# aarchiiive/diff-unet-amos

Hardware: AMD Instinct MI355X
Metric: denoised voxel-steps/sec on 96^3 16-class AMOS patches (higher is better)
Workload: dtype f16

## Files before the change

diff_unet_amos_amd/_native.py:

```python
from __future__ import annotations

import ctypes as C
import os

import torch

_HERE = os.path.dirname(os.path.abspath(__file__))
LIB_PATH = os.path.join(_HERE, "libdua_hip.so")
if os.environ.get("DUA_DEBUG") == "1" and os.environ.get("DUA_HIP_LIB"):
    LIB_PATH = os.environ["DUA_HIP_LIB"]

F32, F16 = 0, 1
U8 = 2
ERR_ARG = -22
SURFACE_FIELDS = ("hd", "hd95", "asd", "assd", "tp", "fp", "fn", "tn", "hd95_lo", "hd95_hi", "asd_ba", "n_surface")


class NativeLibraryMissing(RuntimeError):
    pass


class Conv3Desc(C.Structure):
    _fields_ = [("dtype", C.c_int), ("N", C.c_int), ("D", C.c_int), ("H", C.c_int), ("W", C.c_int),
                ("Cin", C.c_int), ("Cin_stride", C.c_int), ("Cin_off", C.c_int),
# ... 71 lines not shown
                ("out", C.c_void_p), ("ldc", C.c_int), ("out_off", C.c_int), ("x", C.c_void_p),
                ("stats", C.c_void_p), ("c_pad", C.c_int), ("geom", WindowGeom), ("gamma", C.c_void_p), ("beta", C.c_void_p),
                ("eps", C.c_float), ("ln_out", C.c_void_p), ("background", C.c_int)]


TOKLIN_PLAIN, TOKLIN_GELU, TOKLIN_STATS, TOKLIN_RESIDUAL, TOKLIN_SCATTER = range(5)

TEMB_MAX_BLOCKS, ADAMW_MAX_TENSORS = 16, 64


class TembBlocks(C.Structure):
    _fields_ = [("nblocks", C.c_int), ("cout", C.c_int * TEMB_MAX_BLOCKS), ("w", C.c_void_p * TEMB_MAX_BLOCKS),
                ("b", C.c_void_p * TEMB_MAX_BLOCKS), ("dw", C.c_void_p * TEMB_MAX_BLOCKS), ("db", C.c_void_p * TEMB_MAX_BLOCKS)]


class PackItem(C.Structure):
    _fields_ = [("kind", C.c_int), ("Cout", C.c_int), ("Cin", C.c_int), ("packed", C.c_int), ("w", C.c_void_p), ("out", C.c_void_p)]


class AdamWList(C.Structure):
    _fields_ = [("count", C.c_int), ("numel", C.c_long * ADAMW_MAX_TENSORS), ("p", C.c_void_p * ADAMW_MAX_TENSORS),
                ("g", C.c_void_p * ADAMW_MAX_TENSORS), ("m", C.c_void_p * ADAMW_MAX_TENSORS), ("v", C.c_void_p * ADAMW_MAX_TENSORS)]

class AugVolume(C.Structure):
    _fields_ = [("image", C.c_void_p), ("label", C.c_void_p), ("fg_prefix", C.c_void_p), ("bg_prefix", C.c_void_p),
                ("D", C.c_int), ("H", C.c_int), ("W", C.c_int), ("nchunks", C.c_int), ("fg_count", C.c_uint),
                ("bg_count", C.c_uint), ("image_threshold", C.c_float), ("reserved", C.c_int)]


class AugConfig(C.Structure):
    _fields_ = [("roi", C.c_int * 3), ("max_k", C.c_int), ("pos_fraction", C.c_float), ("flip_prob", C.c_float),
                ("rot90_prob", C.c_float), ("scale_prob", C.c_float), ("scale_factors", C.c_float), ("shift_prob", C.c_float),
                ("shift_offsets", C.c_float), ("reserved", C.c_int)]


class AugSmoothing(C.Structure):
    _fields_ = [("alpha", C.c_float), ("order", C.c_float), ("epsilon", C.c_float), ("max_value", C.c_float)]


AUG_CHUNK, AUG_MAX_CLASSES, AUG_PARAM_WORDS = 1024, 64, 8
AUG_VOLUME, AUG_START_D, AUG_START_H, AUG_START_W, AUG_FLIP, AUG_K, AUG_SCALE, AUG_SHIFT = range(8)

_P = C.c_void_p
ABI_VERSION = 8

_SIGS = {
    "dua_abi_version": (C.c_int, []),
    "dua_prepare": (C.c_int, []),
    "dua_prepared_kernels": (C.c_int, []),
    "dua_mfma_probe": (C.c_int, [C.c_int, C.c_int, _P, _P, _P]),
    "dua_chain_probe": (C.c_int, [C.c_int, C.c_int, _P, _P, _P, _P]),
    "dua_deconv_k2s2_fwd": (C.c_int, [C.POINTER(Conv3Desc), _P, _P, _P, C.POINTER(InNorm), _P, _P]),
    "dua_deconv_k2s2_pad_fwd": (C.c_int, [C.POINTER(Conv3Desc), C.c_int, C.c_int, C.c_int, _P, _P, _P, C.POINTER(InNorm), _P, _P]),
    "dua_conv3d_k3_dgrad_reduce_supported": (C.c_int, [C.POINTER(Conv3Desc)]),
    "dua_conv3d_k3_dgrad_reduce": (C.c_int, [C.POINTER(Conv3Desc), _P, _P, _P, _P, _P, C.c_int, C.c_int, C.POINTER(InNorm), _P, _P]),
    "dua_deconv_k2s2_res_supported": (C.c_int, [C.POINTER(Conv3Desc), C.c_int]),
    "dua_deconv_k2s2_res_fwd": (C.c_int, [C.POINTER(Conv3Desc), _P, _P, _P, C.c_int, C.c_int, C.c_int, _P, _P, _P, _P]),
    "dua_q_sample": (C.c_int, [C.c_int, C.c_long, _P, _P, _P, _P, _P]),
    "dua_sampler_step": (C.c_int, [C.c_int, C.c_int, C.c_long, _P, _P, _P, _P, _P, _P, _P, _P]),
    "dua_final_conv_sampler": (C.c_int, [C.POINTER(TailDesc), _P, C.POINTER(InNorm)] + [_P] * 11),
    "dua_final_conv_sampler_res": (C.c_int, [C.POINTER(TailDesc), _P, C.POINTER(InNorm), C.POINTER(TailResidual)] + [_P] * 11),
    "dua_window_attention_fwd": (C.c_int, [C.c_int, C.c_int, C.c_int, C.c_int, C.c_int, _P, _P, _P, _P, _P, C.c_int, C.c_int, C.c_int,
                                           C.c_float, _P, _P]),
    "dua_patch_merge_norm": (C.c_int, [C.c_int] * 7 + [_P, _P, _P, _P, C.c_float, _P, _P]),
    "dua_residual_norm_act": (C.c_int, [C.c_int, C.c_int, C.c_long, C.c_int, _P, C.c_int, C.POINTER(InNorm), _P, C.c_int,
                                        C.POINTER(InNorm), _P, C.c_int, C.c_int, C.c_float, _P, C.c_int, C.c_int, _P, C.c_int,
                                        C.c_int, C.c_int, _P]),
    "dua_window_gather_norm": (C.c_int, [C.c_int, C.POINTER(WindowGeom), _P, _P, _P, _P, C.c_float, _P, _P]),
    "dua_window_scatter_add_norm": (C.c_int, [C.c_int, C.POINTER(WindowGeom), _P, _P, _P, _P, C.c_float, _P, _P]),
    "dua_stage_out": (C.c_int, [C.c_int, C.c_int, C.c_long, C.c_int, _P, _P, C.c_int, C.c_float, _P, _P, _P, C.c_int, C.c_int, _P]),
    "dua_patch_embed": (C.c_int, [C.c_int] * 8 + [_P, _P, _P, _P, C.c_int, C.c_float, _P, _P, _P, C.c_int, C.c_int, _P]),
    "dua_instnorm_stats": (C.c_int, [C.c_int, C.c_int, C.c_long, C.c_int, _P, C.c_int, C.c_int, _P, C.c_int, _P]),
    "dua_gelu": (C.c_int, [C.c_int, C.c_long, _P, _P]),
    "dua_token_linear": (C.c_int, [C.POINTER(TokenLinearDesc), _P]),
    "dua_token_gemm": (C.c_int, [C.POINTER(TokenLinearDesc), _P, C.c_long, _P]),
    "dua_token_gemm_workspace": (C.c_long, [C.c_long, C.c_int, C.c_int]),
    "dua_swin_mlp": (C.c_int, [C.c_long, C.c_int, _P, _P, _P, _P, _P, _P, _P]),
    "dua_denoiser_step": (C.c_int, [C.POINTER(DenoiserPlan), _P]),
    "dua_temb_table": (C.c_int, [C.c_int, _P, _P, C.c_int, C.c_int, _P, _P, _P, _P, _P, _P, C.c_int, _P, _P]),
    "dua_step_begin": (C.c_int, [C.c_int, C.c_int, _P, C.c_int, _P, _P, C.c_int, _P, _P, _P, _P, _P, _P, _P]),
    "dua_step_begin_clear": (C.c_int, [C.c_int, C.c_int, _P, C.c_int, _P, _P, C.c_int, _P, _P, _P, _P, _P, _P, _P, C.c_long, _P]),
    "dua_conv3d_k3_workspace": (C.c_long, [C.POINTER(Conv3Desc)]),
    "dua_conv3d_k3_kernel_kind": (C.c_int, [C.POINTER(Conv3Desc), C.c_int, C.c_int]),
    "dua_deconv_k2s2_kernel_kind": (C.c_int, [C.POINTER(Conv3Desc)]),
    "dua_conv3d_k3_fwd": (C.c_int, [C.POINTER(Conv3Desc), _P, _P, _P, C.POINTER(InNorm), _P, _P, _P, C.c_long, _P]),
    "dua_upconv_k3_supported": (C.c_int, [C.POINTER(UpConvDesc)]),
    "dua_pack_upconv_weights": (C.c_long, [C.c_int, C.c_int, C.c_int, C.c_int, C.c_int, C.c_int, _P, _P, _P, _P, _P, _P, _P]),
    "dua_upconv_k3_fwd": (C.c_int, [C.POINTER(UpConvDesc), _P, _P, C.POINTER(InNorm), _P, _P, _P, _P, _P, _P]),
    "dua_conv3d_k3_wgrad_workspace": (C.c_long, [C.POINTER(Conv3Desc)]),
    "dua_conv3d_k3_wgrad": (C.c_int, [C.POINTER(Conv3Desc), _P, _P, _P, C.c_int, _P, _P, C.c_long, _P]),
    "dua_pack_conv3_weights": (C.c_long, [C.c_int, C.c_int, C.c_int, C.c_int, _P, _P, _P, _P]),
    "dua_pack_conv3_weights_tap": (C.c_long, [C.c_int, C.c_int, C.c_int, C.c_int, C.c_int, C.c_int, _P, _P, _P, _P]),
    "dua_pack_conv3_weights_dgrad": (C.c_long, [C.c_int, C.c_int, C.c_int, C.c_int, _P, _P, _P]),
    "dua_instnorm_finalize": (C.c_int, [C.c_int, C.c_int, C.POINTER(InNorm), _P, _P, _P]),
    "dua_instnorm_bwd_reduce": (C.c_int, [C.POINTER(NormBwdDesc), _P, _P, C.POINTER(InNorm), _P, _P]),
    "dua_instnorm_bwd_apply": (C.c_int, [C.POINTER(NormBwdDesc), _P, _P, C.POINTER(InNorm), _P, _P, _P, _P, _P, _P]),
    "dua_maxpool2_bwd_add": (C.c_int, [C.c_int] * 6 + [_P, C.c_int, C.c_int, _P, C.c_int, C.c_int, _P, C.c_int, _P, C.c_int, _P]),
    "dua_pack_deconv_weights_dgrad": (C.c_long, [C.c_int, C.c_int, C.c_int, _P, _P, _P]),
    "dua_deconv_k2s2_bwd_workspace": (C.c_long, [C.POINTER(Conv3Desc)]),
    "dua_deconv_k2s2_bwd": (C.c_int, [C.POINTER(Conv3Desc), _P, _P, _P, _P, _P, _P, C.c_long, _P]),
    "dua_deconv_k2s2_pad_bwd": (C.c_int, [C.POINTER(Conv3Desc), C.c_int, C.c_int, C.c_int, _P, _P, _P, _P, _P, _P, C.c_long, _P]),
    "dua_head_fwd": (C.c_int, [C.c_int, C.c_long, C.c_int, C.c_int, _P, C.c_int, _P, _P, _P, C.c_int, _P]),
    "dua_head_bwd_workspace": (C.c_long, [C.c_long]),
    "dua_head_bwd": (C.c_int, [C.c_int, C.c_long, C.c_int, C.c_int, _P, C.c_int, _P, C.c_int, _P, _P, C.c_int, _P, _P, _P, C.c_long, _P]),
    "dua_seg_loss_reduce": (C.c_int, [C.c_int, C.c_int, C.c_int, C.c_long, _P, C.c_int, _P, _P, _P]),
    "dua_seg_loss_grad": (C.c_int, [C.c_int, C.c_int, C.c_int, C.c_long, _P, C.c_int, _P, _P, _P, C.c_float, C.c_float,
                                    C.c_float, _P, C.c_int, _P]),
    "dua_materialize": (C.c_int, [C.POINTER(MaterializeDesc), _P, C.POINTER(InNorm), _P, _P, _P, _P]),
    "dua_pack_deconv_weights": (C.c_long, [C.c_int, C.c_int, C.c_int, _P, _P, _P]),
    "dua_to_channels_last": (C.c_int, [C.c_int, C.c_int, C.c_int, C.c_long, _P, _P, C.c_int, C.c_int, C.c_int, _P]),
    "dua_from_channels_last": (C.c_int, [C.c_int, C.c_int, C.c_int, C.c_long, _P, C.c_int, C.c_int, _P, _P]),
    "dua_pack_conv3_weights_batch": (C.c_int, [C.c_int, C.c_int, C.POINTER(PackItem), _P]),
    "dua_to_channels_last_rows": (C.c_int, [C.c_int, C.c_int, C.c_int, _P, C.c_int, _P, C.c_long, _P, C.c_int, _P]),
    "dua_linear_f32": (C.c_int, [C.c_long, C.c_int, C.c_int, _P, C.c_long, _P, _P, _P, C.c_long, C.c_int, _P]),
    "dua_stats_channel_sums": (C.c_int, [C.c_int, C.c_int, C.c_int, _P, _P, _P]),
    "dua_seg_loss_finish": (C.c_int, [C.c_int, C.c_int, C.c_long, C.c_int, C.c_int, C.c_int, C.c_int, _P, _P, _P, _P]),
    "dua_q_sample_affine": (C.c_int, [C.c_int, C.c_long, _P, C.c_float, C.c_float, _P, _P, C.c_int, _P, _P, _P]),
    "dua_multi_neighbor_columns": (C.c_int, [C.c_int] * 7 + [_P, C.c_int, _P, _P, _P]),
    "dua_multi_neighbor_angles": (C.c_int, [C.c_int, C.c_int, _P, _P, _P]),
    "dua_seg_loss_finish_mn": (C.c_int, [C.c_int, C.c_int, C.c_long, C.c_int, C.c_int, C.c_int, C.c_int, _P, C.c_int, _P, _P, _P,
                                         _P]),
    "dua_temb_train_fwd": (C.c_int, [C.c_int, _P, _P, C.c_int, C.c_int, _P, _P, _P, _P, C.POINTER(TembBlocks), _P, _P, _P]),
    "dua_temb_train_bwd": (C.c_int, [C.c_int, C.c_int, C.c_int, _P, C.POINTER(TembBlocks), _P, _P, _P, _P, _P, _P, _P, _P]),
    "dua_grads_nonfinite": (C.c_int, [C.POINTER(AdamWList), _P, _P]),
    "dua_adamw_step": (C.c_int, [C.POINTER(AdamWList), C.c_float, _P, C.c_float, C.c_float, C.c_float, C.c_float, _P, _P, _P,
                                 C.c_int, _P]),
    "dua_adamw_advance": (C.c_int, [_P, _P, _P, _P, C.c_float, C.c_float, C.c_int, _P, _P]),
    "dua_surface_scratch_bytes": (C.c_long, [C.c_int] * 4),
    "dua_surface_masks": (C.c_int, [C.c_int] * 4 + [_P, C.c_int, C.c_long, _P, C.c_int, C.c_long, C.c_int, _P, C.c_long, _P, _P]),
    "dua_surface_edt_sq": (C.c_int, [C.c_int] * 4 + [_P, C.c_long, C.c_int, C.c_double, C.c_double, C.c_double, _P, _P]),
    "dua_surface_distance_table": (C.c_int, [C.c_int] * 4 + [_P, C.c_int, C.c_long, _P, C.c_int, C.c_long, C.c_int] +
                                   [C.c_double] * 3 + [C.c_int, _P, _P, _P, C.c_long, _P]),
    "dua_aug_count_candidates": (C.c_int, [_P, _P, C.c_long, C.c_float, _P, _P]),
    "dua_aug_draw": (C.c_int, [_P, C.c_int, _P, C.c_int, C.POINTER(AugConfig), C.c_ulonglong, _P, C.c_int, C.c_ulonglong, _P, _P,
                               _P]),
    "dua_aug_apply": (C.c_int, [_P, C.c_int, _P, C.c_int, C.c_int, C.c_int, C.c_int, _P, C.c_int, _P, _P, _P, _P]),
    "dua_aug_class_centroids": (C.c_int, [_P, C.c_int, C.c_int, C.c_int, C.c_int, _P, _P, _P]),
    "dua_aug_apply_smoothed": (C.c_int, [_P, C.c_int, _P, C.c_int, C.POINTER(AugSmoothing), _P, C.c_int, C.c_int, C.c_int, C.c_int,
                                         _P, C.c_int, _P, _P, _P, _P]),
}

_lib = None


def exported_symbols():
    return sorted(_SIGS)


def lib():
    global _lib
    if _lib is None:
        if not os.path.exists(LIB_PATH):
            raise NativeLibraryMissing(
                f"{LIB_PATH} not found: build it with `python -c 'import __graft_entry__ as g; g.build()'` "
                "(hipcc --offload-arch=gfx950). There is no CPU fallback.")
        L = C.CDLL(LIB_PATH)
        for name, (res, args) in _SIGS.items():
            fn = getattr(L, name)
            fn.restype, fn.argtypes = res, args
        got = L.dua_abi_version()
        if got != ABI_VERSION:
            raise NativeLibraryMissing(f"{LIB_PATH} has ABI version {got}, this binding needs {ABI_VERSION}: rebuild the library")
        _lib = L
    return _lib


# ... 29 lines not shown
```

diff_unet_amos_amd/csrc/conv3d_igemm.hip:

```cpp
#include "common.hpp"
#include "../../include/dua_hip.h"
#include "conv3_args.hpp"
#include "stamp.hpp"
#include <algorithm>

namespace dua {

namespace c3 {
constexpr int TD = 4, TH = 8, TW = 8;
constexpr int HD = TD + 2, HH = TH + 2, HW = TW + 2;
constexpr int KG = 4;
constexpr int VS = KG * 16;
constexpr int RS = HW * VS + 16;
constexpr int PS = HH * RS;
constexpr int HALO_BYTES = HD * PS;
constexpr int BN = 64;
}

static inline int conv_variant_of(const dua_conv3_desc* d) { return d->policy & 0xff; }
static inline bool conv_policy_ok(const dua_conv3_desc* d) {
  const int v = d->policy & 0xff;
  return (d->policy & ~(0xff | DUA_POLICY_NO_FINISH)) == 0 && (v == 0 || v == 2 || v == 3 || v == 6 || v == 7 || v == 8 || v == 9);
}

#ifdef DUA_ABLATE
extern int g_wgrad_abl;
#endif

namespace c3v2 {
using namespace c3;
constexpr int SLAB = 3 * KG * BN * 16;
constexpr int LDS_MAIN = HALO_BYTES + 2 * SLAB;
}

__device__ __forceinline__ void glds16(const void* g, void* lds_wave_base) {
  __builtin_amdgcn_global_load_lds((const __attribute__((address_space(1))) void*)g,
                                   (__attribute__((address_space(3))) void*)lds_wave_base, 16, 0, 0);
}

template <typename T, int TDP = 4, int NKS = 2, bool HALF = false, bool BIG = false>
__global__ __launch_bounds__(256, BIG ? 1 : 2) void conv3d_k3_v2_kernel(Conv3Args a) {
  using namespace c3v2;
  constexpr int TD = TDP, HD = TDP + 2, MB = TDP == 2 ? 1 : 2;
  constexpr int NW = 4, NTHR = 64 * NW;
  constexpr int BSLAB = 3 * SLAB;
  constexpr int HALO_BYTES = HD * PS, LDS_MAIN = HALO_BYTES + (BIG ? 3 * BSLAB : 2 * SLAB);
  static_assert(!BIG || (NKS == 2 && !HALF), "the kd-plane form is the plain 32-channel-chunk kernel");
  constexpr int NITEMS = HD * HH * HW * KG, NIT = (NITEMS + NTHR - 1) / NTHR;
  constexpr int NPIECE = SLAB / 16, NSL = (NPIECE + NTHR - 1) / NTHR;
  using Frag = typename Elem<T>::Frag;
  constexpr int EPG = Elem<T>::EPG;
  constexpr int CK = KG * EPG;
  extern __shared__ __attribute__((aligned(16))) char smem[];
  char* halo = smem;
  char* wbuf = smem + HALO_BYTES;
  float* xsc = (float*)(smem + LDS_MAIN);
  float* xsh = xsc + a.nchunks * CK;
  float* xad = xsh + a.nchunks * CK;

  const int tid = threadIdx.x, lane = tid & 63, wave = tid >> 6;
  const int r = lane & 31, hh = lane >> 5;
  const int dwave = TDP == 2 ? wave >> 1 : wave;
  const int hbase = TDP == 2 ? (wave & 1) * 4 : 0;
  const int tile = xcd_remap(blockIdx.x, a.ntiles);
  const int ct = blockIdx.y, n = blockIdx.z % a.N;
  const int tw_ = tile % a.tiles_w, th_ = (tile / a.tiles_w) % a.tiles_h, td_ = tile / (a.tiles_w * a.tiles_h);
  const int d0 = td_ * TD, h0 = th_ * TH, w0 = tw_ * TW;
  const bool fused = a.xf.stats != nullptr;

  const int kg_t = tid & (KG - 1);
  long goff[NIT]; int loff[NIT];
  const T* xin = (const T*)a.x + (long)n * a.D * a.H * a.W * a.Cin_stride + a.Cin_off;
#pragma unroll
  for (int j = 0; j < NIT; ++j) {
    int it = tid + NTHR * j;
    int hv = it >> 2;
    int hd = hv / (HH * HW), rem = hv - hd * (HH * HW), hy = rem / HW, hx = rem - hy * HW;
    int gd = d0 + hd - 1, gh = h0 + hy - 1, gw = w0 + hx - 1;
    bool ok = it < NITEMS && gd >= 0 && gd < a.D && gh >= 0 && gh < a.H && gw >= 0 && gw < a.W;
    goff[j] = ok ? (((long)gd * a.H + gh) * a.W + gw) * a.Cin_stride + kg_t * EPG : -1;
#ifndef DUA_HALO_BRANCHFREE
    loff[j] = it < NITEMS ? hd * PS + hy * RS + hx * VS + kg_t * 16 : -1;
#else
    loff[j] = it < NITEMS ? hd * PS + hy * RS + hx * VS + kg_t * 16 : HW * VS;
#endif
  }
  const char* wsrc = (const char*)a.w + (long)ct * a.nchunks * 9 * SLAB;
  f32x4 wreg[3][NSL];
  auto load_slab = [&](int g, int set) {
    const char* src = wsrc + (long)g * SLAB + tid * 16;
#pragma unroll
    for (int j = 0; j < NSL; ++j)
      if (NPIECE % NTHR == 0 || tid + NTHR * j < NPIECE) wreg[set][j] = *(const f32x4*)(src + j * NTHR * 16);
  };
  auto store_slab = [&](int g, int set) {
    char* dst = wbuf + (g & 1) * SLAB + tid * 16;
#pragma unroll
    for (int j = 0; j < NSL; ++j)
      if (NPIECE % NTHR == 0 || tid + NTHR * j < NPIECE) *(f32x4*)(dst + j * NTHR * 16) = wreg[set][j];
  };
  Frag hv_[NIT];
#ifndef DUA_HALO_BRANCHFREE
  auto load_halo = [&](int ch) {
    const bool cok = ch * CK + kg_t * EPG < a.Cin;
#pragma unroll
// ... 518 lines not shown
        mma32(acc[m][0], ta[m][s], tb[s][0]);
        mma32(acc[m][1], ta[m][s], tb[s][1]);
      }
    if (slot < 56) DUA_STAMP_AT(slot, false);
    __syncthreads();
    if (slot < 56) DUA_STAMP_AT(slot + 1, false);

    char* ot = halo + wave * 4096;
    float* ex = (float*)(smem + LDS_F);
    const int gd = d0 + wave;
    const bool dok = gd < a.D;
    const bool full = d0 + TD <= a.D && h0 + TH <= a.H && w0 + TW <= a.W;
    const long nvox = (long)a.D * a.H * a.W;
    T* yout = (T*)a.y + (long)n * nvox * a.Cout_stride;
    float s[2] = {0.f, 0.f}, ss[2] = {0.f, 0.f};
#pragma unroll
    for (int m = 0; m < MB; ++m) {
      if (full) {
#pragma unroll
        for (int q = 0; q < 2; ++q)
#pragma unroll
          for (int i = 0; i < 16; ++i) {
            const float v = acc[m][q][i];
            s[q] += v;
            ss[q] = fmaf(v, v, ss[q]);
            *(T*)(ot + acc_row(i, hh) * 128 + (q * 32 + r) * 2) = (T)v;
          }
      } else {
#pragma unroll
        for (int q = 0; q < 2; ++q)
#pragma unroll
          for (int i = 0; i < 16; ++i) {
            const int hl = 4 * m + (i >> 2), wl = (i & 3) + 4 * hh;
            const bool ok = dok && (h0 + hl < a.H) && (w0 + wl < a.W);
            const float v = ok ? acc[m][q][i] : 0.f;
            s[q] += v;
            ss[q] = fmaf(v, v, ss[q]);
            *(T*)(ot + acc_row(i, hh) * 128 + (q * 32 + r) * 2) = (T)v;
          }
      }
      __builtin_amdgcn_fence(__ATOMIC_RELEASE, "wavefront");
      __builtin_amdgcn_wave_barrier();
      __builtin_amdgcn_fence(__ATOMIC_ACQUIRE, "wavefront");
      if (dok) {
#pragma unroll
        for (int it = 0; it < 4; ++it) {
          const int v = it * 8 + (lane >> 3), cg = lane & 7;
          const int gh = h0 + 4 * m + (v >> 3), gw = w0 + (v & 7);
          if ((full || (gh < a.H && gw < a.W)) && ct * BN + cg * 8 < a.Cout)
            *(f16x8*)(yout + chan_off(a.out_blk, ((long)gd * a.H + gh) * a.W + gw, a.Cout_off + ct * BN + cg * 8, a.Cout_stride, nvox)) =
                *(const f16x8*)(ot + v * 128 + cg * 16);
        }
      }
      __builtin_amdgcn_fence(__ATOMIC_RELEASE, "wavefront");
      __builtin_amdgcn_wave_barrier();
      __builtin_amdgcn_fence(__ATOMIC_ACQUIRE, "wavefront");
    }
#pragma unroll
    for (int q = 0; q < 2; ++q) {
      s[q] += __shfl_xor(s[q], 32);
      ss[q] += __shfl_xor(ss[q], 32);
      if (hh == 0) { ex[(wave * BN + q * 32 + r) * 2] = s[q]; ex[(wave * BN + q * 32 + r) * 2 + 1] = ss[q]; }
    }
    if (slot < 56) DUA_STAMP_AT(slot + 2, false);
    __syncthreads();
    if (wave == 0) {
      double S = 0, Q = 0;
#pragma unroll
      for (int w = 0; w < NW; ++w) { S += (double)ex[(w * BN + lane) * 2]; Q += (double)ex[(w * BN + lane) * 2 + 1]; }
      if (ct * BN + lane < a.Cout) stats_add(a.stats, n, a.cout_pad, item & (STAT_REPLICAS - 1), ct * BN + lane, S, Q);
    }
    if (more) {
      store_halo();
      __syncthreads();
    }
    if (slot < 56) DUA_STAMP_AT(slot + 3, false);
    slot += 4;
  }
  DUA_STAMP_AT(62, false);
  DUA_STAMP_AT(63, false);
  DUA_STAMP_AT(1, true);
}

template <typename T>
__global__ __launch_bounds__(256) void splitk_finish_kernel(const float* __restrict__ part, int ksplit, int N, long vox,
                                                            int cout_pad, int Cout, const float* __restrict__ bias,
                                                            T* __restrict__ y, int Cout_stride, int Cout_off,
                                                            stat_t* stats, int G, int VL, int ITER) {
  using part_t = typename std::conditional<sizeof(T) == 4, double, float>::type;
  __shared__ part_t red[256][8];
  const int n = blockIdx.y;
  const int cg = threadIdx.x % G, vl = threadIdx.x / G;
  const int c = cg * 4;
  part_t s[4] = {0, 0, 0, 0}, q[4] = {0, 0, 0, 0};
  f32x4 b4 = {0.f, 0.f, 0.f, 0.f};
  if (c < Cout) b4 = *(const f32x4*)(bias + c);
  if (vl < VL && ITER == 2 && ksplit <= 8) {
    const long va = ((long)blockIdx.x * 2) * VL + vl, vb = va + VL;
    const long kstride = (long)N * vox * cout_pad;
    const float* pa = part + ((long)n * vox + (va < vox ? va : 0)) * cout_pad + c;
    const float* pb = part + ((long)n * vox + (vb < vox ? vb : 0)) * cout_pad + c;
    f32x4 qa[8], qb[8];
#pragma unroll
    for (int j = 0; j < 8; ++j) {
      const int kk = j < ksplit ? j : ksplit - 1;
      qa[j] = *(const f32x4*)(pa + kk * kstride);
      qb[j] = *(const f32x4*)(pb + kk * kstride);
    }
    f32x4 acc[2] = {b4, b4};
#pragma unroll
    for (int j = 0; j < 8; ++j)
      if (j < ksplit)
#pragma unroll
        for (int e = 0; e < 4; ++e) { acc[0][e] += qa[j][e]; acc[1][e] += qb[j][e]; }
#pragma unroll
    for (int i = 0; i < 2; ++i) {
      const long v = i ? vb : va;
      if (v >= vox) break;
      T o[4];
#pragma unroll
      for (int e = 0; e < 4; ++e) {
        o[e] = (T)acc[i][e];
        const float f = (float)o[e];
        s[e] += f; q[e] += (part_t)f * (part_t)f;
      }
      if (c < Cout) {
        T* yp = y + ((long)n * vox + v) * Cout_stride + Cout_off + c;
#pragma unroll
        for (int e = 0; e < 4; ++e) yp[e] = o[e];
      }
    }
  } else if (vl < VL) {
    for (int i = 0; i < ITER; ++i) {
      const long v = ((long)blockIdx.x * ITER + i) * VL + vl;
      if (v >= vox) break;
      f32x4 acc = b4;
      const float* pp = part + ((long)n * vox + v) * cout_pad + c;
      const long kstride = (long)N * vox * cout_pad;
      int k = 0;
      for (; k + 16 <= ksplit; k += 16) {
        f32x4 pv[16];
#pragma unroll
        for (int j = 0; j < 16; ++j) pv[j] = *(const f32x4*)(pp + (k + j) * kstride);
#pragma unroll
        for (int j = 0; j < 16; ++j)
#pragma unroll
          for (int e = 0; e < 4; ++e) acc[e] += pv[j][e];
      }
      if (k < ksplit) {
        f32x4 pv[16];
#pragma unroll
        for (int j = 0; j < 16; ++j) {
          const int kk = k + j < ksplit ? k + j : ksplit - 1;
          pv[j] = *(const f32x4*)(pp + kk * kstride);
        }
#pragma unroll
        for (int j = 0; j < 16; ++j)
          if (k + j < ksplit)
#pragma unroll
            for (int e = 0; e < 4; ++e) acc[e] += pv[j][e];
      }
      T o[4];
#pragma unroll
      for (int e = 0; e < 4; ++e) {
        o[e] = (T)acc[e];
        const float f = (float)o[e];
        s[e] += f; q[e] += (part_t)f * (part_t)f;
      }
      if (c < Cout) {
        T* yp = y + ((long)n * vox + v) * Cout_stride + Cout_off + c;
#pragma unroll
        for (int e = 0; e < 4; ++e) yp[e] = o[e];
      }
    }
  }
#pragma unroll
  for (int e = 0; e < 4; ++e) { red[threadIdx.x][e] = s[e]; red[threadIdx.x][4 + e] = q[e]; }
  __syncthreads();
  for (int ch = threadIdx.x; ch < 4 * G; ch += 256) {
    const int g4 = ch >> 2, e = ch & 3;
    double S = 0, Q = 0;
    for (int j = 0; j < VL; ++j) { S += (double)red[j * G + g4][e]; Q += (double)red[j * G + g4][4 + e]; }
    if (ch < Cout) stats_add(stats, n, cout_pad, blockIdx.x & (STAT_REPLICAS - 1), ch, S, Q);
  }
}


static inline void choose_split(int base_wgs, int units, int* ksplit, int* ups, int target = 320, int max_base = 64) {
  *ksplit = 1; *ups = units;
  if (base_wgs > max_base || units <= 1) return;
  int want = target == 320 ? (320 + base_wgs - 1) / base_wgs : target / base_wgs;
  if (want < 1) want = 1;
  if (want > units) want = units;
  *ups = (units + want - 1) / want;
  *ksplit = (units + *ups - 1) / *ups;
}

constexpr int PARTIAL_LDS_PAD = 36 * 1024;

static const LdsAttr kConvLdsAttrs[] = {
    {(const void*)conv3d_k3_v2_kernel<f16, 4>, c3v2::LDS_MAIN + 3 * 4 * 1024 + PARTIAL_LDS_PAD},
    {(const void*)conv3d_k3_v2_kernel<float, 4>, c3v2::LDS_MAIN + 3 * 4 * 1024 + PARTIAL_LDS_PAD},
    {(const void*)conv3d_k3_v2_kernel<f16, 4, 1>, c3v2::LDS_MAIN + 4096 + PARTIAL_LDS_PAD},
    {(const void*)conv3d_k3_v2_kernel<f16, 4, 0>, c3v2::LDS_MAIN + 4096 + PARTIAL_LDS_PAD},
    {(const void*)conv3d_k3_v2_kernel<f16, 4, 2, true>, c3v2::LDS_MAIN + 3 * 4 * 1024 + PARTIAL_LDS_PAD},
    {(const void*)conv3d_k3_first_kernel, c3f::LDS_F + 2048 + PARTIAL_LDS_PAD},
    {(const void*)conv3d_k3_v2_kernel<f16, 2>, c3v2::LDS_MAIN + 3 * 4 * 1024},
    {(const void*)conv3d_k3_v2_kernel<float, 2>, c3v2::LDS_MAIN + 3 * 4 * 1024},
    {(const void*)conv3d_k3_v2_kernel<f16, 4, 2, false, true>, 160 * 1024},
    {(const void*)conv3d_k3_v2_kernel<float, 4, 2, false, true>, 160 * 1024},
    {(const void*)conv3d_k3_v2_kernel<f16, 2, 2, false, true>, 160 * 1024},
    {(const void*)conv3d_k3_v2_kernel<float, 2, 2, false, true>, 160 * 1024},
};
static const LdsAttrs kConvLdsReg(kConvLdsAttrs);

static int conv3_kernel_kind(const dua_conv3_desc* d, bool fused) {
  const int g_conv_variant = conv_variant_of(d);
  if (d->dtype != DUA_F16) return 0;
  if (d->tap_channel_plus1 > 0) return (d->tap_channel_plus1 == 17 && g_conv_variant == 0) ? 1 : 0;
  const long tiles = (long)((d->D + 3) / 4) * ((d->H + 7) / 8) * ((d->W + 7) / 8) * ((d->Cout + c3::BN - 1) / c3::BN) * d->N;
  const long vox = (long)d->D * d->H * d->W;
  if ((g_conv_variant == 0 || g_conv_variant == 8 || g_conv_variant == 9) && !d->background && tiles >= 1024 && d->D % 8 == 0 && d->H % 8 == 0 && d->W % 8 == 0 &&
      d->Cin % 16 == 0 && d->Cin <= (fused ? 256 : 384) && vox * d->Cin_stride < 0x7fffffffL)
    return 2;
  return 0;
}

struct BwdSums { const void* raw; int stride, off; const dua_in_norm* in; double* sums; };

template <typename T>
static int launch_conv3(const dua_conv3_desc* d, const void* x, const void* w, const float* bias,
                        const dua_in_norm* in, void* y, stat_t* stats, float* ws, long ws_bytes, hipStream_t s,
                        const BwdSums* bw = nullptr) {
  using namespace c3;
  constexpr int CK = KG * Elem<T>::EPG;
  Conv3Args a;
  a.x = x; a.w = w; a.bias = bias; a.y = y; a.stats = stats;
  a.bw_raw = nullptr; a.bw_stride = a.bw_off = 0; a.bw_xf = make_xform(nullptr, d->Cout); a.bw_sums = nullptr;
  if (bw) {
    a.bw_raw = bw->raw; a.bw_stride = bw->stride; a.bw_off = bw->off; a.bw_xf = make_xform(bw->in, d->Cout); a.bw_sums = bw->sums;
  }
  a.xf = make_xform(in, d->Cin);
  a.N = d->N; a.D = d->D; a.H = d->H; a.W = d->W;
  a.Cin = d->Cin; a.Cin_stride = d->Cin_stride; a.Cin_off = d->Cin_off;
  a.Cout = d->Cout; a.Cout_stride = d->Cout_stride; a.Cout_off = d->Cout_off;
  a.nchunks = (d->Cin + CK - 1) / CK;
  const int td = (d->D + TD - 1) / TD;
  a.tiles_h = (d->H + TH - 1) / TH; a.tiles_w = (d->W + TW - 1) / TW;
  a.ntiles = td * a.tiles_h * a.tiles_w;
  const int nct = (d->Cout + BN - 1) / BN;
  a.cout_pad = nct * BN;
  a.ksplit = 1; a.units_per_split = a.nchunks * 3; a.part = nullptr; a.tap_ch = -1;
  a.in_blk = d->layout & DUA_IN_BLOCKED ? 1 : 0; a.out_blk = d->layout & DUA_OUT_BLOCKED ? 1 : 0;
  if (a.nchunks * CK > 1024 || !conv_policy_ok(d)) return DUA_ERR_ARG;
  const int g_conv_variant = conv_variant_of(d);
  const int kind = conv3_kernel_kind(d, in && in->stats);
  if ((a.in_blk && kind != 2) || (a.out_blk && kind == 0)) return DUA_ERR_ARG;
  if ((a.in_blk && (d->Cin_off % 16 || d->Cin_stride % 16)) || (a.out_blk && (d->Cout_off % 16 || d->Cout_stride % 16))) return DUA_ERR_ARG;
  const int xf_bytes = in && in->stats ? 3 * 4 * a.nchunks * CK : 0;
  if (int e = ensure_prepared()) return e;
  const long vox = (long)d->D * d->H * d->W;
  const int bg_pad = d->background ? PARTIAL_LDS_PAD : 0;
  if (d->tap_channel_plus1 > 0) {
    a.tap_ch = d->tap_channel_plus1 - 1;
    if constexpr (sizeof(T) != 2) return DUA_ERR_ARG;
    else {
      if (a.nchunks != 1 || (in && in->stats) || (a.tap_ch != 0 && a.tap_ch != 16) || d->Cin != a.tap_ch + 8) return DUA_ERR_ARG;
      dim3 grid(a.ntiles, nct, d->N);
      if (kind == 1) {
        const int cus = device_cus();
        if (cus <= 0) return DUA_ERR_ARG;
        const int items = a.ntiles * d->N;
        const int wgs = std::max(1, (bg_pad ? 1 : 2) * cus / nct);
        hipLaunchKernelGGL(conv3d_k3_first_kernel, dim3(std::min(items, wgs), nct, 1), dim3(256), c3f::LDS_F + 2048 + bg_pad, s, a, items);
        return (int)hipGetLastError();
      }
      if (a.tap_ch == 16) hipLaunchKernelGGL((conv3d_k3_v2_kernel<T, 4, 1>), grid, dim3(256), c3v2::LDS_MAIN + 4096 + bg_pad, s, a);
      else hipLaunchKernelGGL((conv3d_k3_v2_kernel<T, 4, 0>), grid, dim3(256), c3v2::LDS_MAIN + 4096 + bg_pad, s, a);
      return (int)hipGetLastError();
    }
  }
  if constexpr (sizeof(T) == 2) {
    if (kind == 2) return launch_conv3_wide(a, d->D, s, g_conv_variant >= 8, g_conv_variant == 9 ? 2 : 0);
  }
  if (bw) return DUA_ERR_ARG;
  const bool autop = g_conv_variant == 0 || g_conv_variant == 2 || g_conv_variant == 6 || g_conv_variant == 7 || g_conv_variant >= 8;
  const bool big = g_conv_variant == 0 || g_conv_variant == 2 || g_conv_variant == 7 || g_conv_variant >= 8;
  if (ws != nullptr && autop) {
    int ks, ups;
    if (g_conv_variant == 2) choose_split(a.ntiles * nct * d->N, a.nchunks * 3, &ks, &ups, 512, 256);
    else choose_split(a.ntiles * nct * d->N, a.nchunks * 3, &ks, &ups, big ? 256 : 320);
    if (ks > 1 && (long)ks * d->N * vox * a.cout_pad * 4 <= ws_bytes) { a.ksplit = ks; a.units_per_split = ups; a.part = ws; }
  }
  if (a.ksplit == 1 && ((autop && a.ntiles * nct * d->N < 200 && a.ntiles * nct * d->N > 64) || g_conv_variant == 3)) {
    const int td2 = (d->D + 1) / 2;
    a.ntiles = td2 * a.tiles_h * a.tiles_w;
    dim3 grid2(a.ntiles, nct, d->N);
    constexpr int LDS2 = 4 * c3::HH * c3::RS + 2 * c3v2::SLAB;
    const bool big2 = big && (long)a.ntiles * nct * d->N <= 256;
    if (big2) hipLaunchKernelGGL((conv3d_k3_v2_kernel<T, 2, 2, false, true>), grid2, dim3(256), 4 * c3::HH * c3::RS + 9 * c3v2::SLAB + xf_bytes, s, a);
    else hipLaunchKernelGGL((conv3d_k3_v2_kernel<T, 2>), grid2, dim3(256), LDS2 + xf_bytes, s, a);
    return (int)hipGetLastError();
  }
  dim3 grid(a.ntiles, nct, d->N * a.ksplit);
  if (a.ksplit > 1) {
    if (big) hipLaunchKernelGGL((conv3d_k3_v2_kernel<T, 4, 2, false, true>), grid, dim3(256), c3::HALO_BYTES + 9 * c3v2::SLAB + xf_bytes, s, a);
    else hipLaunchKernelGGL(conv3d_k3_v2_kernel<T>, grid, dim3(256), c3v2::LDS_MAIN + xf_bytes, s, a);
    if (d->policy & DUA_POLICY_NO_FINISH) return (int)hipGetLastError();
    const int G = a.cout_pad / 4 > 256 ? 256 : a.cout_pad / 4;
    if (a.cout_pad / 4 > 256) return DUA_ERR_ARG;
    const int VL = 256 / G;
    int ITER = 8;
    while (ITER > 1 && (vox + (long)VL * ITER - 1) / ((long)VL * ITER) < 128) ITER >>= 1;
    dim3 fgrid((unsigned)((vox + (long)VL * ITER - 1) / ((long)VL * ITER)), d->N);
    hipLaunchKernelGGL(splitk_finish_kernel<T>, fgrid, dim3(256), 0, s, (const float*)ws, a.ksplit, d->N, vox, a.cout_pad,
                       d->Cout, bias, (T*)y, d->Cout_stride, d->Cout_off, stats, G, VL, ITER);
    return (int)hipGetLastError();
  }
  if (sizeof(T) == 2 && d->Cin - (a.nchunks - 1) * CK <= CK / 2)
    hipLaunchKernelGGL((conv3d_k3_v2_kernel<T, 4, 2, true>), grid, dim3(256), c3v2::LDS_MAIN + xf_bytes + bg_pad, s, a);
  else
    hipLaunchKernelGGL(conv3d_k3_v2_kernel<T>, grid, dim3(256), c3v2::LDS_MAIN + xf_bytes + bg_pad, s, a);
  return (int)hipGetLastError();
}

}

extern "C" {

#ifdef DUA_STAMP
long dua_debug_stamps(void* host, long bytes) { return dua::stamps_out(host, bytes); }
#endif

#ifdef DUA_ABLATE
int dua_set_option(int key, int value) {
  if (key == 3 && value >= 0 && value < 16) { dua::g_wgrad_abl = value; return 0; }
  return DUA_ERR_ARG;
}
#endif

int dua_conv3d_k3_kernel_kind(const dua_conv3_desc* d, int fused, int has_workspace) {
  if (!d || !dua::conv_policy_ok(d)) return DUA_ERR_ARG;
  (void)has_workspace;
  return dua::conv3_kernel_kind(d, fused != 0);
}

long dua_conv3d_k3_workspace(const dua_conv3_desc* d) {
  using namespace dua::c3;
  if (!d || (d->dtype != DUA_F16 && d->dtype != DUA_F32)) return DUA_ERR_ARG;
  const int ck = 4 * (d->dtype == DUA_F16 ? 8 : 4);
  const int nch = (d->Cin + ck - 1) / ck, nct = (d->Cout + BN - 1) / BN;
  const int tiles = ((d->D + TD - 1) / TD) * ((d->H + TH - 1) / TH) * ((d->W + TW - 1) / TW);
  int ks, ups;
  dua::choose_split(tiles * nct * d->N, nch * 3, &ks, &ups);
  return ks > 1 ? (long)ks * d->N * d->D * d->H * d->W * nct * BN * 4 : 0;
}

int dua_conv3d_k3_fwd(const dua_conv3_desc* d, const void* x, const void* w_packed, const float* bias_padded,
                      const dua_in_norm* in, void* y, dua_stat_word* out_stats, void* workspace, long workspace_bytes,
                      void* stream) {
  if (!d || !x || !w_packed || !bias_padded || !y || !out_stats) return DUA_ERR_ARG;
  if (d->Cin % 8 || d->Cout % 8 || d->Cin_stride % 8 || d->Cout_stride % 8 || d->Cin_off % 8 || d->Cout_off % 8)
    return DUA_ERR_ARG;
  if (in && in->stats && (!in->gamma || !in->beta || in->c_pad < d->Cin || in->count <= 0 || !(in->slope >= 0.f && in->slope <= 1.f))) return DUA_ERR_ARG;
  if (d->dtype == DUA_F16)
    return dua::launch_conv3<dua::f16>(d, x, w_packed, bias_padded, in, y, out_stats, (float*)workspace, workspace_bytes, (hipStream_t)stream);
  if (d->dtype == DUA_F32)
    return dua::launch_conv3<float>(d, x, w_packed, bias_padded, in, y, out_stats, (float*)workspace, workspace_bytes, (hipStream_t)stream);
  return DUA_ERR_ARG;
}

int dua_conv3d_k3_dgrad_reduce_supported(const dua_conv3_desc* d) {
  if (!d || d->dtype != DUA_F16 || d->layout || d->tap_channel_plus1 || d->background || dua::conv_variant_of(d) != 0) return 0;
  return dua::conv3_kernel_kind(d, false) == 2 ? 1 : 0;
}

int dua_conv3d_k3_dgrad_reduce(const dua_conv3_desc* d, const void* dy, const void* w_packed, const float* bias_padded, void* dx,
                               const void* raw, int raw_stride, int raw_off, const dua_in_norm* raw_in, double* sums, void* stream) {
  if (!dua_conv3d_k3_dgrad_reduce_supported(d) || !dy || !w_packed || !bias_padded || !dx || !raw || !raw_in || !sums) return DUA_ERR_ARG;
  if (d->Cin % 8 || d->Cout % 8 || d->Cin_stride % 8 || d->Cout_stride % 8 || d->Cin_off % 8 || d->Cout_off % 8) return DUA_ERR_ARG;
  if (!raw_in->stats || !raw_in->gamma || !raw_in->beta || raw_in->c_pad < d->Cout || raw_in->count <= 0 ||
      !(raw_in->slope >= 0.f && raw_in->slope <= 1.f) || raw_stride % 8 || raw_off % 8 || raw_off + d->Cout > raw_stride)
    return DUA_ERR_ARG;
  const dua::BwdSums bw{raw, raw_stride, raw_off, raw_in, sums};
  return dua::launch_conv3<dua::f16>(d, dy, w_packed, bias_padded, nullptr, dx, nullptr, nullptr, 0, (hipStream_t)stream, &bw);
}

}
```

include/dua_hip.h:

```cpp
#ifndef DUA_HIP_H
#define DUA_HIP_H
#ifdef __cplusplus
extern "C" {
#endif

#define DUA_F32 0
#define DUA_F16 1
#define DUA_ERR_ARG (-22)

typedef long long dua_stat_word;
typedef struct {
  const dua_stat_word* stats;
  const float* gamma;
  const float* beta;
  const float* add;
  int add_stride;
  int c_pad;
  long long count;
  float eps;
  float slope;
} dua_in_norm;

typedef struct {
  int dtype;
  int N, D, H, W;
  int Cin, Cin_stride, Cin_off;
  int Cout, Cout_stride, Cout_off;
  int tap_channel_plus1;
  int background;
  int layout;
  int policy;
} dua_conv3_desc;
#define DUA_POLICY_NO_FINISH 256
#define DUA_IN_BLOCKED 1
#define DUA_OUT_BLOCKED 2

int dua_conv3d_k3_kernel_kind(const dua_conv3_desc* d, int fused, int has_workspace);
int dua_deconv_k2s2_kernel_kind(const dua_conv3_desc* d);

long dua_conv3d_k3_workspace(const dua_conv3_desc* d);
int dua_conv3d_k3_fwd(const dua_conv3_desc* d, const void* x, const void* w_packed, const float* bias_padded,
                      const dua_in_norm* in, void* y, dua_stat_word* out_stats, void* workspace, long workspace_bytes,
                      void* stream);

typedef struct {
  int dtype;
  int N, D, H, W;
  int Cskip, Cskip_stride, Cskip_off;
  int Cu, Cu_stride, Cu_off;
  int Cout, Cout_stride, Cout_off;
  int layout;
} dua_upconv_desc;
int dua_upconv_k3_supported(const dua_upconv_desc* d);
long dua_pack_upconv_weights(int dtype, int Cout, int Cskip, int Cmid, int Cu, int up_first, const float* wc, const float* bc,
                             const float* wd, const float* bd, void* wu_packed, float* bias_table, void* stream);
int dua_upconv_k3_fwd(const dua_upconv_desc* d, const void* xskip, const void* u, const dua_in_norm* u_in, const void* w_skip_packed,
                      const void* wu_packed, const float* bias_table, void* y, dua_stat_word* out_stats, void* stream);

long dua_conv3d_k3_wgrad_workspace(const dua_conv3_desc* d);
long dua_pack_conv3_weights_dgrad(int dtype, int Cout, int Cin, int Cout_packed, const float* w, void* w_packed,
                                  void* stream);
int dua_conv3d_k3_wgrad(const dua_conv3_desc* d, const void* x, const void* dy, float* dw, int Cin_src,
                        const int* in_perm, void* workspace, long workspace_bytes, void* stream);

typedef struct {
  int dtype;
  int N;
  long voxels;
  int C;
  int da_stride, da_off;
  int raw_stride, raw_off;
  int out_stride, out_off;
} dua_norm_bwd_desc;
int dua_instnorm_bwd_reduce(const dua_norm_bwd_desc* d, const void* dA, const void* raw, const dua_in_norm* in,
                            double* sums, void* stream);
int dua_instnorm_bwd_apply(const dua_norm_bwd_desc* d, const void* dA, const void* raw, const dua_in_norm* in,
                           const double* sums, void* dY, float* dgamma, float* dbeta, float* dadd, void* stream);

int dua_conv3d_k3_dgrad_reduce_supported(const dua_conv3_desc* d);
int dua_conv3d_k3_dgrad_reduce(const dua_conv3_desc* d, const void* dy, const void* w_packed, const float* bias_padded, void* dx,
                               const void* raw, int raw_stride, int raw_off, const dua_in_norm* raw_in, double* sums, void* stream);

int dua_deconv_k2s2_res_supported(const dua_conv3_desc* d, int Cs);
int dua_deconv_k2s2_res_fwd(const dua_conv3_desc* d, const void* lo, const void* w_packed, const void* xskip, int Cs, int Cs_stride,
                            int Cs_off, const void* ws_packed, void* y, dua_stat_word* stats, void* stream);

int dua_maxpool2_bwd_add(int dtype, int N, int D, int H, int W, int C, const void* act, int act_stride, int act_off,
                         const void* dA, int da_stride, int da_off, const void* dP, int dp_stride, void* out,
                         int out_stride, void* stream);

long dua_pack_deconv_weights_dgrad(int dtype, int Cin, int Cout, const float* w, void* w_packed, void* stream);
long dua_deconv_k2s2_bwd_workspace(const dua_conv3_desc* d);
int dua_deconv_k2s2_bwd(const dua_conv3_desc* d, const void* x, const void* dy, const void* w_packed_dgrad, void* dx,
                        float* dw, void* workspace, long workspace_bytes, void* stream);
int dua_deconv_k2s2_pad_bwd(const dua_conv3_desc* d, int Do, int Ho, int Wo, const void* x, const void* dy,
                            const void* w_packed_dgrad, void* dx, float* dw, void* workspace, long workspace_bytes, void* stream);

int dua_head_fwd(int dtype, long voxels, int C, int K, const void* u, int u_stride, const float* W, const float* b,
                 void* logits, int logits_stride, void* stream);
long dua_head_bwd_workspace(long voxels);
int dua_head_bwd(int dtype, long voxels, int C, int K, const void* dlogits, int dlogits_stride, const void* u,
                 int u_stride, const float* W, void* du, int du_stride, float* dW, float* db, void* workspace,
                 long workspace_bytes, void* stream);

int dua_seg_loss_reduce(int dtype, int N, int C, long voxels, const void* logits, int logits_stride, const float* labels,
                        double* sums, void* stream);
int dua_seg_loss_grad(int dtype, int N, int C, long voxels, const void* logits, int logits_stride, const float* labels,
                      const double* sums, const float* gscale, float w_mse, float w_bce, float w_dice, void* dlogits,
                      int dlogits_stride, void* stream);

int dua_stats_channel_sums(int N, int C, int c_pad, const dua_stat_word* stats, float* out, void* stream);
int dua_seg_loss_finish(int N, int C, long voxels, int use_mse, int use_bce, int use_dice, int combine, const double* sums,
                        float* loss, float* dcomb, void* stream);
int dua_q_sample_affine(int N, long per_sample, const float* src, float a, float b, const float* eps, const float* sched, int T,
                        const long long* t, float* out, void* stream);

int dua_multi_neighbor_columns(int dtype, int N, int C, int K, int D, int H, int W, const void* logits, int logits_stride,
                               const float* labels, unsigned long long* csums, void* stream);
int dua_multi_neighbor_angles(int N, int K, const unsigned long long* csums, double* partials, void* stream);
int dua_seg_loss_finish_mn(int N, int C, long voxels, int use_mse, int use_bce, int use_dice, int K, const double* mn_partials,
                           int combine, const double* sums, float* loss, float* dcomb, void* stream);

#define DUA_TEMB_MAX_BLOCKS 16
// ... 305 lines not shown
```

Before: 681.5 million.

## Add specialised split-K conv3d kernel for the 12x12x12 bottleneck level

Result: no change. 686.4 million (median of 6 runs) (+0.7%).

```diff
diff --git a/diff_unet_amos_amd/_native.py b/diff_unet_amos_amd/_native.py
--- a/diff_unet_amos_amd/_native.py
+++ b/diff_unet_amos_amd/_native.py
@@ -177,6 +177,7 @@
     "dua_step_begin_clear": (C.c_int, [C.c_int, C.c_int, _P, C.c_int, _P, _P, C.c_int, _P, _P, _P, _P, _P, _P, _P, C.c_long, _P]),
     "dua_conv3d_k3_workspace": (C.c_long, [C.POINTER(Conv3Desc)]),
     "dua_conv3d_k3_kernel_kind": (C.c_int, [C.POINTER(Conv3Desc), C.c_int, C.c_int]),
+    "dua_conv3d_k3_level_form": (C.c_int, [C.POINTER(Conv3Desc), C.c_long]),
     "dua_deconv_k2s2_kernel_kind": (C.c_int, [C.POINTER(Conv3Desc)]),
     "dua_conv3d_k3_fwd": (C.c_int, [C.POINTER(Conv3Desc), _P, _P, _P, C.POINTER(InNorm), _P, _P, _P, C.c_long, _P]),
     "dua_upconv_k3_supported": (C.c_int, [C.POINTER(UpConvDesc)]),
diff --git a/diff_unet_amos_amd/csrc/conv3d_igemm.hip b/diff_unet_amos_amd/csrc/conv3d_igemm.hip
--- a/diff_unet_amos_amd/csrc/conv3d_igemm.hip
+++ b/diff_unet_amos_amd/csrc/conv3d_igemm.hip
@@ -20,7 +20,7 @@
 static inline int conv_variant_of(const dua_conv3_desc* d) { return d->policy & 0xff; }
 static inline bool conv_policy_ok(const dua_conv3_desc* d) {
   const int v = d->policy & 0xff;
-  return (d->policy & ~(0xff | DUA_POLICY_NO_FINISH)) == 0 && (v == 0 || v == 2 || v == 3 || v == 6 || v == 7 || v == 8 || v == 9);
+  return (d->policy & ~(0xff | DUA_POLICY_NO_FINISH)) == 0 && (v == 0 || v == 2 || v == 3 || v == 6 || v == 7 || v == 8 || v == 9 || v == 10);
 }
 
 #ifdef DUA_ABLATE
@@ -705,6 +705,175 @@
   DUA_STAMP_AT(1, true);
 }
 
+namespace c3l {
+using c3::KG; using c3::VS; using c3::BN;
+constexpr int BD = 4, BH = 12, BW = 4;
+constexpr int MB = 3;
+constexpr int RSB = 25 * 16, PSB = 352 * 16;
+constexpr int NP = BD + 2, NR = BH + 2, NC = BW + 2;
+constexpr int LHALO = NP * PSB;
+constexpr int LPLANE = 3 * c3v2::SLAB;
+constexpr int LDS_STATIC = LHALO + 3 * LPLANE;
+}
+
+__global__ __launch_bounds__(256, 1) void conv3d_k3_level_kernel(Conv3Args a) {
+  using namespace c3l;
+  using T = f16;
+  using Frag = f16x8;
+  constexpr int NTHR = 256, EPG = 8, CK = KG * EPG;
+  constexpr int NITEMS = NP * NR * NC * KG, NIT = (NITEMS + NTHR - 1) / NTHR;
+  __shared__ __attribute__((aligned(16))) char lds[LDS_STATIC];
+  extern __shared__ __attribute__((aligned(16))) char smem[];
+  char* halo = lds;
+  char* wbuf = lds + LHALO;
+  float* xsc = (float*)smem;
+  float* xsh = xsc + a.nchunks * CK;
+  float* xad = xsh + a.nchunks * CK;
+
+  const int tid = threadIdx.x, lane = tid & 63, wave = tid >> 6;
+  const int r = lane & 31, hh = lane >> 5;
+  const int mh = wave >> 1, q = wave & 1;
+  const int boxes_d = a.D / BD;
+  const int d0 = (blockIdx.x % boxes_d) * BD, w0 = (blockIdx.x / boxes_d) * BW;
+  const int ct = blockIdx.y, ks_id = blockIdx.z;
+  const bool fused = a.xf.stats != nullptr;
+
+  const int kg_t = tid & (KG - 1);
+  long goff[NIT]; int loff[NIT];
+  const T* xin = (const T*)a.x + a.Cin_off;
+#pragma unroll
+  for (int j = 0; j < NIT; ++j) {
+    const int it = tid + NTHR * j;
+    const int hv = it >> 2;
+    const int p = hv / (NR * NC), rem = hv - p * (NR * NC), hy = rem / NC, hx = rem - hy * NC;
+    const int gd = d0 + p - 1, gh = hy - 1, gw = w0 + hx - 1;
+    const bool ok = it < NITEMS && gd >= 0 && gd < a.D && gh >= 0 && gh < a.H && gw >= 0 && gw < a.W;
+    goff[j] = ok ? (((long)gd * a.H + gh) * a.W + gw) * a.Cin_stride + kg_t * EPG : -1;
+    loff[j] = it < NITEMS ? p * PSB + hy * RSB + hx * VS + kg_t * 16 : -1;
+  }
+  const char* wsrc = (const char*)a.w + (long)ct * a.nchunks * 9 * c3v2::SLAB;
+  Frag hv_[NIT];
+  auto load_halo = [&](int ch) {
+#pragma unroll
+    for (int j = 0; j < NIT; ++j) {
+      if (goff[j] >= 0) hv_[j] = *(const Frag*)(xin + goff[j] + ch * CK);
+      else
+#pragma unroll
+        for (int e = 0; e < EPG; ++e) hv_[j][e] = (T)0.f;
+    }
+  };
+  auto store_halo = [&](int ch) {
+    const int c0 = ch * CK + kg_t * EPG;
+    if (fused) {
+      float sc[EPG], sh[EPG], ad[EPG], sn[EPG];
+#pragma unroll
+      for (int e = 0; e < EPG; ++e) { sc[e] = xsc[c0 + e]; sh[e] = xsh[c0 + e]; ad[e] = xad[c0 + e]; }
+      xform_prep<T>(sc, sh, ad, sn, a.xf.slope);
+#pragma unroll
+      for (int j = 0; j < NIT; ++j)
+        if (goff[j] >= 0) hv_[j] = xform_frag<T>(hv_[j], sc, sh, ad, sn, a.xf.slope);
+    }
+#pragma unroll
+    for (int j = 0; j < NIT; ++j)
+      if (loff[j] >= 0) *(Frag*)(halo + loff[j]) = hv_[j];
+  };
+  auto dma_unit = [&](int u, int slot) {
+    const char* src = wsrc + (long)u * LPLANE + (wave * 9) * 1024 + lane * 16;
+    const unsigned dst = (unsigned)(size_t)(__attribute__((address_space(3))) char*)(wbuf + slot * LPLANE + (wave * 9) * 1024);
+#pragma unroll
+    for (int j = 0; j < 9; ++j) {
+      unsigned keep;
+      asm volatile("s_mov_b32 %0, m0\n\ts_mov_b32 m0, %2\n\ts_nop 0\n\tglobal_load_lds_dwordx4 %1, off\n\ts_mov_b32 m0, %0"
+                   : "=&s"(keep) : "v"(src + j * 1024), "s"(__builtin_amdgcn_readfirstlane(dst + j * 1024)) : "memory");
+    }
+  };
+
+  f32x16 acc[MB];
+#pragma unroll
+  for (int m = 0; m < MB; ++m)
+#pragma unroll
+    for (int i = 0; i < 16; ++i) acc[m][i] = 0.f;
+  const int u0 = ks_id * a.units_per_split;
+  const int u1 = min(a.nchunks * 3, u0 + a.units_per_split);
+
+  DUA_STAMP_AT(0, true);
+  DUA_STAMP_AT(2, false);
+  load_halo(u0 / 3);
+  dma_unit(u0, 0);
+  if (u0 + 1 < u1) dma_unit(u0 + 1, 1);
+  DUA_STAMP_AT(59, false);
+  if (fused) {
+    xform_preamble(a.xf, 0, min(a.Cin, ((u1 + 2) / 3) * CK), xsc, xsh, xad, (u0 / 3) * CK);
+    __syncthreads();
+  }
+  DUA_STAMP_AT(60, false);
+  DUA_STAMP_AT(61, false);
+  store_halo(u0 / 3);
+  asm volatile("s_waitcnt vmcnt(0)" ::: "memory");
+  __syncthreads();
+  DUA_STAMP_AT(3, false);
+
+  int a_off[MB];
+#pragma unroll
+  for (int m = 0; m < MB; ++m) {
+    const int line = (mh * MB + m) * 8 + (r >> 2);
+    a_off[m] = (line / BH) * PSB + (line % BH) * RSB + (r & 3) * VS + hh * 16;
+  }
+  const int b_base = (hh * BN + q * 32 + r) * 16;
+  constexpr int NTB = 18;
+  for (int u = u0; u < u1; ++u) {
+    const int kd = u % 3, slot = (u - u0) % 3;
+    const bool next_chunk = kd == 2 && u + 1 < u1;
+    if (next_chunk) load_halo(u / 3 + 1);
+    const bool ahead = u + 2 < u1;
+    if (ahead) dma_unit(u + 2, (u - u0 + 2) % 3);
+    const char* ap = halo + kd * PSB;
+    const char* wb = wbuf + slot * LPLANE + b_base;
+    Frag fa[MB][2], fb[2];
+    auto ldb = [&](int t, int b) {
+      const int tap = t / 2, ks = t % 2, kh = tap / 3, kw = tap % 3;
+#pragma unroll
+      for (int m = 0; m < MB; ++m) fa[m][b] = *(const Frag*)(ap + a_off[m] + kh * RSB + kw * VS + ks * 32);
+      fb[b] = *(const Frag*)(wb + (tap * KG + 2 * ks) * BN * 16);
+    };
+    ldb(0, 0);
+#pragma unroll
+    for (int t = 0; t < NTB; ++t) {
+      if (t + 1 < NTB) ldb(t + 1, (t + 1) & 1);
+      __builtin_amdgcn_sched_barrier(0);
+#pragma unroll
+      for (int m = 0; m < MB; ++m) mma32(acc[m], fa[m][t & 1], fb[t & 1]);
+      __builtin_amdgcn_sched_barrier(0);
+    }
+    if (ahead) asm volatile("s_waitcnt vmcnt(9)" ::: "memory");
+    else asm volatile("s_waitcnt vmcnt(0)" ::: "memory");
+    __syncthreads();
+    if (u - u0 < 55) DUA_STAMP_AT(4 + (u - u0), false);
+    if (next_chunk) {
+      store_halo(u / 3 + 1);
+      __syncthreads();
+    }
+  }
+  DUA_STAMP_AT(62, false);
+  constexpr int OSF = 32 * 4 + 16;
+  char* otf = lds + wave * (32 * MB) * OSF;
+  float* pout = a.part + ((long)ks_id * a.D * a.H * a.W) * a.cout_pad + ct * BN + q * 32;
+#pragma unroll
+  for (int m = 0; m < MB; ++m)
+#pragma unroll
+    for (int i = 0; i < 16; ++i) *(float*)(otf + (m * 32 + acc_row(i, hh)) * OSF + r * 4) = acc[m][i];
+  __syncthreads();
+#pragma unroll
+  for (int it = 0; it < 4 * MB; ++it) {
+    const int row = it * 8 + (lane >> 3), cg = lane & 7;
+    const int line = mh * MB * 8 + (row >> 2);
+    const int gd = d0 + line / BH, gh = line % BH, gw = w0 + (row & 3);
+    *(f32x4*)(pout + (((long)gd * a.H + gh) * a.W + gw) * a.cout_pad + cg * 4) = *(const f32x4*)(otf + row * OSF + cg * 16);
+  }
+  DUA_STAMP_AT(63, false);
+  DUA_STAMP_AT(1, true);
+}
+
 template <typename T>
 __global__ __launch_bounds__(256) void splitk_finish_kernel(const float* __restrict__ part, int ksplit, int N, long vox,
                                                             int cout_pad, int Cout, const float* __restrict__ bias,
@@ -819,6 +988,27 @@
   *ksplit = (units + *ups - 1) / *ups;
 }
 
+static inline int conv3_split_of(const dua_conv3_desc* d, long ws_bytes, int* ups) {
+  using namespace c3;
+  const int v = conv_variant_of(d);
+  const int nch = (d->Cin + (d->dtype == DUA_F16 ? 31 : 15)) / (d->dtype == DUA_F16 ? 32 : 16), nct = (d->Cout + BN - 1) / BN;
+  const int tiles = ((d->D + TD - 1) / TD) * ((d->H + TH - 1) / TH) * ((d->W + TW - 1) / TW);
+  *ups = nch * 3;
+  const bool autop = v == 0 || v == 2 || v == 6 || v == 7 || v >= 8;
+  const bool big = v == 0 || v == 2 || v == 7 || v >= 8;
+  if (ws_bytes <= 0 || !autop) return 1;
+  int ks, u;
+  if (v == 2) choose_split(tiles * nct * d->N, nch * 3, &ks, &u, 512, 256);
+  else choose_split(tiles * nct * d->N, nch * 3, &ks, &u, big ? 256 : 320);
+  if (ks > 1 && (long)ks * d->N * d->D * d->H * d->W * nct * BN * 4 <= ws_bytes) { *ups = u; return ks; }
+  return 1;
+}
+
+static inline bool conv3_level_form(const dua_conv3_desc* d, int ks) {
+  return d->dtype == DUA_F16 && conv_variant_of(d) == 0 && ks > 1 && d->N == 1 && !d->background && !d->layout && !d->tap_channel_plus1 &&
+         d->D == 12 && d->H == c3l::BH && d->W == 12 && d->Cin % 32 == 0;
+}
+
 constexpr int PARTIAL_LDS_PAD = 36 * 1024;
 
 static const LdsAttr kConvLdsAttrs[] = {
@@ -840,10 +1030,10 @@
 static int conv3_kernel_kind(const dua_conv3_desc* d, bool fused) {
   const int g_conv_variant = conv_variant_of(d);
   if (d->dtype != DUA_F16) return 0;
-  if (d->tap_channel_plus1 > 0) return (d->tap_channel_plus1 == 17 && g_conv_variant == 0) ? 1 : 0;
+  if (d->tap_channel_plus1 > 0) return (d->tap_channel_plus1 == 17 && (g_conv_variant == 0 || g_conv_variant == 10)) ? 1 : 0;
   const long tiles = (long)((d->D + 3) / 4) * ((d->H + 7) / 8) * ((d->W + 7) / 8) * ((d->Cout + c3::BN - 1) / c3::BN) * d->N;
   const long vox = (long)d->D * d->H * d->W;
-  if ((g_conv_variant == 0 || g_conv_variant == 8 || g_conv_variant == 9) && !d->background && tiles >= 1024 && d->D % 8 == 0 && d->H % 8 == 0 && d->W % 8 == 0 &&
+  if ((g_conv_variant == 0 || g_conv_variant >= 8) && !d->background && tiles >= 1024 && d->D % 8 == 0 && d->H % 8 == 0 && d->W % 8 == 0 &&
       d->Cin % 16 == 0 && d->Cin <= (fused ? 256 : 384) && vox * d->Cin_stride < 0x7fffffffL)
     return 2;
   return 0;
@@ -904,16 +1094,15 @@
     }
   }
   if constexpr (sizeof(T) == 2) {
-    if (kind == 2) return launch_conv3_wide(a, d->D, s, g_conv_variant >= 8, g_conv_variant == 9 ? 2 : 0);
+    if (kind == 2) return launch_conv3_wide(a, d->D, s, g_conv_variant == 8 || g_conv_variant == 9, g_conv_variant == 9 ? 2 : 0);
   }
   if (bw) return DUA_ERR_ARG;
   const bool autop = g_conv_variant == 0 || g_conv_variant == 2 || g_conv_variant == 6 || g_conv_variant == 7 || g_conv_variant >= 8;
   const bool big = g_conv_variant == 0 || g_conv_variant == 2 || g_conv_variant == 7 || g_conv_variant >= 8;
-  if (ws != nullptr && autop) {
-    int ks, ups;
-    if (g_conv_variant == 2) choose_split(a.ntiles * nct * d->N, a.nchunks * 3, &ks, &ups, 512, 256);
-    else choose_split(a.ntiles * nct * d->N, a.nchunks * 3, &ks, &ups, big ? 256 : 320);
-    if (ks > 1 && (long)ks * d->N * vox * a.cout_pad * 4 <= ws_bytes) { a.ksplit = ks; a.units_per_split = ups; a.part = ws; }
+  {
+    int ups;
+    const int ks = conv3_split_of(d, ws != nullptr ? ws_bytes : 0, &ups);
+    if (ks > 1) { a.ksplit = ks; a.units_per_split = ups; a.part = ws; }
   }
   if (a.ksplit == 1 && ((autop && a.ntiles * nct * d->N < 200 && a.ntiles * nct * d->N > 64) || g_conv_variant == 3)) {
     const int td2 = (d->D + 1) / 2;
@@ -927,7 +1116,9 @@
   }
   dim3 grid(a.ntiles, nct, d->N * a.ksplit);
   if (a.ksplit > 1) {
-    if (big) hipLaunchKernelGGL((conv3d_k3_v2_kernel<T, 4, 2, false, true>), grid, dim3(256), c3::HALO_BYTES + 9 * c3v2::SLAB + xf_bytes, s, a);
+    if (conv3_level_form(d, a.ksplit))
+      hipLaunchKernelGGL(conv3d_k3_level_kernel, dim3((d->D / c3l::BD) * (d->W / c3l::BW), nct, a.ksplit), dim3(256), xf_bytes, s, a);
+    else if (big) hipLaunchKernelGGL((conv3d_k3_v2_kernel<T, 4, 2, false, true>), grid, dim3(256), c3::HALO_BYTES + 9 * c3v2::SLAB + xf_bytes, s, a);
     else hipLaunchKernelGGL(conv3d_k3_v2_kernel<T>, grid, dim3(256), c3v2::LDS_MAIN + xf_bytes, s, a);
     if (d->policy & DUA_POLICY_NO_FINISH) return (int)hipGetLastError();
     const int G = a.cout_pad / 4 > 256 ? 256 : a.cout_pad / 4;
@@ -966,6 +1157,13 @@
   if (!d || !dua::conv_policy_ok(d)) return DUA_ERR_ARG;
   (void)has_workspace;
   return dua::conv3_kernel_kind(d, fused != 0);
+}
+
+int dua_conv3d_k3_level_form(const dua_conv3_desc* d, long workspace_bytes) {
+  if (!d || !dua::conv_policy_ok(d)) return DUA_ERR_ARG;
+  if ((d->dtype != DUA_F16 && d->dtype != DUA_F32) || d->tap_channel_plus1 > 0 || dua::conv3_kernel_kind(d, false) != 0) return 0;
+  int ups;
+  return dua::conv3_level_form(d, dua::conv3_split_of(d, workspace_bytes, &ups)) ? 1 : 0;
 }
 
 long dua_conv3d_k3_workspace(const dua_conv3_desc* d) {
diff --git a/include/dua_hip.h b/include/dua_hip.h
--- a/include/dua_hip.h
+++ b/include/dua_hip.h
@@ -39,6 +39,7 @@
 int dua_deconv_k2s2_kernel_kind(const dua_conv3_desc* d);
 
 long dua_conv3d_k3_workspace(const dua_conv3_desc* d);
+int dua_conv3d_k3_level_form(const dua_conv3_desc* d, long workspace_bytes);
 int dua_conv3d_k3_fwd(const dua_conv3_desc* d, const void* x, const void* w_packed, const float* bias_padded,
                       const dua_in_norm* in, void* y, dua_stat_word* out_stats, void* workspace, long workspace_bytes,
                       void* stream);
```
